# LMP88959/NTSC-CRT

Measured on AMD Instinct MI355X. Metric: frames/sec at 640x480 interlaced, bit-exact vs CPU; % HBM roofline, higher is better.
Workload: dtype int32; 1 GPU; NTSC 640x480 -> 640x480 BGRA, interlaced, full colour, noise 24, hue 0, scanlines 1 (BASELINE configs[1]); mode=independent frames (crthip_fieldpass), launch=eager, batches_in_flight=2

## Files before the change

### ntsc-crt_amd/csrc/crt_decode.hip

```cpp
#include "crt_decode_lane.h"

static int decoder_min_tier(const crthip_ctx *c, const crthip_params *p)
{
    const int b = p->bright < 0 ? -p->bright : p->bright;
    const long ct = p->contrast < 0 ? -(long) p->contrast : (long) p->contrast;
    if (c->force_exact || b > FAST_BRIGHT_MAX || ct >= (1 << 23)) return 3;
    bool coef_ok = p->eq_lf[0] >= 32768 && p->eq_lf[0] < 98304 && p->eq_hf[0] >= 32768 && p->eq_hf[0] < 98304 &&
                   p->eq_lf[1] > 0 && p->eq_lf[1] < 32768 && p->eq_hf[1] > 0 && p->eq_hf[1] < 32768 &&
                   p->eq_lf[2] > 0 && p->eq_lf[2] < 32768 && p->eq_hf[2] > 0 && p->eq_hf[2] < 32768;
    for (int cas = 0; cas < 2 && coef_ok; cas++) {
        const double cf = cas ? p->eq_hf[0] : p->eq_lf[0], al = cf / 65536.0, den = 1.0 - (al > 1.0 ? al - 1.0 : 1.0 - al);
        double prev = 127.0 + b, worst = 0.0;
        for (int k = 0; k < 4; k++) {
            const double cur = (al * prev + 1.0) / den + 1.0;
            if (prev + cur > worst) worst = prev + cur;
            prev = cur;
        }
        if (cf * worst + 32768.0 >= 2147483647.0) coef_ok = false;
    }
    if (c->no_tier0 || !coef_ok || b > T0_BRIGHT_MAX) return 2;
    const long vmax = 16380L * (10L * (127 + b) + 64) + 11551L * 3870L;
    if (((vmax >> 12) + 1) * ct >= (1L << 31)) return 2;
    return c->no_loskip ? 2 : 0;
}
// ... 34 lines not shown
                   const crthip_line *d_lines, void *d_out, size_t ostride, size_t fstride)
{
    if (!fstride) fstride = c->fstride;
    c->last_fstage = 0;
    {
        const int rc = crt_decode_check(c, p);
        if (rc) return rc;
    }
    const bool wide_px = c->px_tile ? c->px_tile >= 32 : p->outw >= 1280;
    const bool rows_shape = !p->eq_kernel && (c->shape == 2 || (c->shape == 0 && n <= ROWS_SHAPE_MAX_FIELDS &&
                            !(n >= WIDE_SHAPE_MIN_FIELDS && !p->bloom && crt_decode_wide_ok(c, p, decoder_min_tier(c, p), wide_px))));
    if (rows_shape) return crt_run_decode_rows(c, p, n, d_inp, d_lines, d_out, ostride, fstride);
    if (p->bloom) return crt_run_decode_bloom_lanes(c, p, n, d_inp, d_lines, d_out, ostride, decoder_min_tier(c, p), fstride);
    const int min_tier = p->eq_kernel ? (decoder_min_tier(c, p) == 3 ? 5 : 4) : decoder_min_tier(c, p);
    const bool wide = wide_px;
    const bool use_wide = crt_decode_wide_ok(c, p, min_tier, wide);
    FStageArgs fsa;
    const bool fstage = crt_decode_fstages(c, p, min_tier, &fsa) && !use_wide;
    c->last_fstage = fstage;
    const unsigned span = (unsigned) p->outh + p->v_fac;
    const int passes = span >= (unsigned) c->sd.lines ? 1 : (int) (((unsigned) c->sd.lines + span - 1) / (span ? span : 1));
    return dispatch_system(c->system, c->pattern, [&](auto tag) {
        using S = decltype(tag);
        {
        const int total = n * S::LINES;
        const block_order bo = make_block_order((total + 63) / 64, c->dec_order_env == -1 ? n : c->dec_order_env);
        const dim3 grid(bo.grid), block(64);
        unsigned char *o = (unsigned char *) d_out;
        ProfScope ps(c, CRTHIP_K_DECODE);
        for (int rank = 0; rank < passes; rank++) {
#define CRTHIP_LAUNCH_DECODE(TG, B3) \
    do { if constexpr (S::CCS != 4 && TG == 2) break;  \
         if constexpr (S::CCS == 4 && TG == 0) { if (fstage) {  \
             if (wide) hipLaunchKernelGGL((k_decode<S, TG, B3, 32, false, true>), grid, block, 0, c->stream, *p, n, d_inp, fstride, d_lines, o, ostride, min_tier, rank, (const int *) nullptr, bo.K, bo.per, fsa); \
             else hipLaunchKernelGGL((k_decode<S, TG, B3, 16, false, true>), grid, block, 0, c->stream, *p, n, d_inp, fstride, d_lines, o, ostride, min_tier, rank, (const int *) nullptr, bo.K, bo.per, fsa); \
             break; } } \
         if (wide) hipLaunchKernelGGL((k_decode<S, TG, B3, 32>), grid, block, 0, c->stream, *p, n, d_inp, fstride, d_lines, o, ostride, min_tier, rank, (const int *) nullptr, bo.K, bo.per, fsa); \
         else hipLaunchKernelGGL((k_decode<S, TG, B3, 16>), grid, block, 0, c->stream, *p, n, d_inp, fstride, d_lines, o, ostride, min_tier, rank, (const int *) nullptr, bo.K, bo.per, fsa); } while (0)
            if (use_wide) {
                const int rc = crt_run_decode_wide(c, p, n, d_inp, d_lines, d_out, ostride, min_tier, rank, fstride);
                if (rc) return rc;
                CRTHIP_LAUNCH_DECODE(1, false);
                continue;
            }
            if (p->out_bpp == 3) {
                if (min_tier <= 1) CRTHIP_LAUNCH_DECODE(0, true);
                if (min_tier <= 3) CRTHIP_LAUNCH_DECODE(1, true);
                if (min_tier >= 4) CRTHIP_LAUNCH_DECODE(2, true);
            } else {
                if (min_tier <= 1) CRTHIP_LAUNCH_DECODE(0, false);
                if (min_tier <= 3) CRTHIP_LAUNCH_DECODE(1, false);
                if (min_tier >= 4) CRTHIP_LAUNCH_DECODE(2, false);
            }
#undef CRTHIP_LAUNCH_DECODE
        }
        return CRTHIP_OK;
        }
    });
}
```

### ntsc-crt_amd/csrc/crt_decode3.hip

```cpp
#include "crt_decode_lane.h"

#define BLOOM_BUCKETS 256
#define BLOOM_KEY_BIAS 64

template <class S>
__device__ __forceinline__ int bloom_key(const crthip_line &lp, int outw)
{
    if ((lp.nrows & CRTHIP_LINE_NROWS_MASK) == 0) return -1;
    const int half = S::AV_LEN / 2 + 8 - (lp.scanl >> 12);
    const int line_w = 2 * half + (lp.dx != ((2 * half) << 12) / outw ? 1 : 0);
    const int key = line_w - S::AV_LEN * 112 / 128 + BLOOM_KEY_BIAS;
    return key < 0 ? 0 : key >= BLOOM_BUCKETS ? BLOOM_BUCKETS - 1 : key;
}

#define BLOOM_SORT_ROUNDS 16

template <class S>
__global__ void __launch_bounds__(256)
k_bloom_count(int total, int outw, const crthip_line *__restrict__ lines, int *__restrict__ hist)
{
    __shared__ int s_hist[BLOOM_BUCKETS];
    const int t = threadIdx.x;
    s_hist[t] = 0;
    __syncthreads();
// ... 67 lines not shown
                               const crthip_line *d_lines, void *d_out, size_t ostride, int min_tier, size_t fstride)
{
    const int total = n * c->sd.lines;
    const size_t slots = bloom_slots(c, n);
    const int rc_ = crt_reserve_bloom(c, n);
    if (rc_) return rc_;
    int *hist = c->d_bloom, *cursor = hist + BLOOM_BUCKETS, *perm = cursor + BLOOM_BUCKETS;
    const bool wide = c->px_tile ? c->px_tile >= 32 : p->outw >= 1280;
    const unsigned span = (unsigned) p->outh + p->v_fac;
    const int passes = span >= (unsigned) c->sd.lines ? 1 : (int) (((unsigned) c->sd.lines + span - 1) / (span ? span : 1));
    if (min_tier == 1 && c->sd.cc_samples != 5) min_tier = 2;
    FStageArgs fsa;
    const bool fstage = crt_decode_fstages(c, p, min_tier, &fsa);
    return dispatch_system(c->system, c->pattern, [&](auto tag) {
        using S = decltype(tag);
        if constexpr (S::NES_TIMING) {
            return set_err(c, CRTHIP_E_ARG, "no bloom build of the NES systems", hipSuccess);
        } else {
            ProfScope ps(c, CRTHIP_K_DECODE);
            {
                const size_t want = (slots + 255) / 256;
                static_assert(2 * BLOOM_BUCKETS <= 256 * 4, "the first blocks clear the histogram and the cursors");
                hipLaunchKernelGGL(k_bloom_clear, dim3((unsigned) (want < 4 ? 4 : want > 2048 ? 2048 : want)), dim3(256), 0, c->stream,
                                   hist, 2 * BLOOM_BUCKETS, perm, slots);
            }
            const dim3 sgrid((total + 256 * BLOOM_SORT_ROUNDS - 1) / (256 * BLOOM_SORT_ROUNDS)), sblock(256);
            hipLaunchKernelGGL((k_bloom_count<S>), sgrid, sblock, 0, c->stream, total, p->outw, d_lines, hist);
            hipLaunchKernelGGL((k_bloom_scatter<S>), sgrid, sblock, 0, c->stream, total, p->outw, d_lines, hist, cursor, perm);
            const dim3 grid((unsigned) (slots / 64)), block(64);
            unsigned char *o = (unsigned char *) d_out;
            for (int rank = 0; rank < passes; rank++) {
#define CRTHIP_LAUNCH_BLOOM(TG, B3) \
    do { if constexpr (S::CCS == 4 && TG == 0) { if (fstage) {  \
             if (wide) hipLaunchKernelGGL((k_decode<S, TG, B3, 32, true, true>), grid, block, 0, c->stream, *p, n, d_inp, fstride, d_lines, o, ostride, min_tier, rank, (const int *) perm, 0, 0, fsa); \
             else hipLaunchKernelGGL((k_decode<S, TG, B3, 16, true, true>), grid, block, 0, c->stream, *p, n, d_inp, fstride, d_lines, o, ostride, min_tier, rank, (const int *) perm, 0, 0, fsa); \
             break; } } \
         if (wide) hipLaunchKernelGGL((k_decode<S, TG, B3, 32, true>), grid, block, 0, c->stream, *p, n, d_inp, fstride, d_lines, o, ostride, min_tier, rank, (const int *) perm, 0, 0, fsa); \
         else hipLaunchKernelGGL((k_decode<S, TG, B3, 16, true>), grid, block, 0, c->stream, *p, n, d_inp, fstride, d_lines, o, ostride, min_tier, rank, (const int *) perm, 0, 0, fsa); } while (0)
                if (p->out_bpp == 3) {
                    if (min_tier <= 1) CRTHIP_LAUNCH_BLOOM(0, true);
                    CRTHIP_LAUNCH_BLOOM(1, true);
                } else {
                    if (min_tier <= 1) CRTHIP_LAUNCH_BLOOM(0, false);
                    CRTHIP_LAUNCH_BLOOM(1, false);
                }
#undef CRTHIP_LAUNCH_BLOOM
            }
            return CRTHIP_OK;
        }
    });
}
```

### ntsc-crt_amd/csrc/crt_decode_lane.h

```cpp
#ifndef CRT_DECODE_LANE_H
#define CRT_DECODE_LANE_H
#include "crt_dev.h"
#include <type_traits>


struct Eq3 { int lo0, lo1, lo2, lo3, hi0, hi1, hi2, hi3, h0, h1, h2; };

template <bool FAST, int G1, int G2>
__device__ __forceinline__ int eq_step(Eq3 &f, const int lf, const int hf, const int s)
{
    f.lo0 += (mulq<FAST>(lf, s - f.lo0) + 32768) >> 16;
    f.hi0 += (mulq<FAST>(hf, s - f.hi0) + 32768) >> 16;
    f.lo1 += (mulq<FAST>(lf, f.lo0 - f.lo1) + 32768) >> 16;
    f.hi1 += (mulq<FAST>(hf, f.hi0 - f.hi1) + 32768) >> 16;
    f.lo2 += (mulq<FAST>(lf, f.lo1 - f.lo2) + 32768) >> 16;
    f.hi2 += (mulq<FAST>(hf, f.hi1 - f.hi2) + 32768) >> 16;
    f.lo3 += (mulq<FAST>(lf, f.lo2 - f.lo3) + 32768) >> 16;
    f.hi3 += (mulq<FAST>(hf, f.hi2 - f.hi3) + 32768) >> 16;
    int r = (f.lo3 * 65536) >> 16;
    if (G1 == 65536 || G1 == 8192) r += ((f.hi3 - f.lo3) * G1) >> 16;
    else r += mulq<FAST>(f.hi3 - f.lo3, G1) >> 16;
    if (G2 != 0) {
        r += mulq<FAST>(f.h2 - f.hi3, G2) >> 16;
        f.h2 = f.h1; f.h1 = f.h0; f.h0 = s;
// ... 58 lines not shown
__device__ __forceinline__ void fstage_round_down(bool on)
{
    __builtin_amdgcn_sched_barrier(0);
    if (on) asm volatile("s_setreg_imm32_b32 hwreg(HW_REG_MODE, 0, 2), 2\n\ts_nop 1" ::: "memory");
    else asm volatile("s_setreg_imm32_b32 hwreg(HW_REG_MODE, 0, 2), 0\n\ts_nop 1" ::: "memory");
    __builtin_amdgcn_sched_barrier(0);
}
__device__ __forceinline__ float fbits(int b) { return __int_as_float(b); }
__device__ __forceinline__ float subf(float a, float b)
{
    float r;
    asm("v_sub_f32 %0, %1, %2" : "=v"(r) : "v"(a), "v"(b));
    return r;
}
__device__ __forceinline__ float fmaf_vs(float d, int m_uniform, float acc)
{
    float r;
    asm("v_fma_f32 %0, %1, %2, %3" : "=v"(r) : "v"(d), "s"(m_uniform), "v"(acc));
    return r;
}
__device__ __forceinline__ float addf_sv(int k_uniform, float x)
{
    float r;
    asm("v_add_f32 %0, %1, %2" : "=v"(r) : "s"(k_uniform), "v"(x));
    return r;
}
template <bool NEG> __device__ __forceinline__ float fmaf_vvs(float a, float b, int k_uniform)
{
    float r;
    if (NEG) asm("v_fma_f32 %0, %1, -%2, %3" : "=v"(r) : "v"(a), "v"(b), "s"(k_uniform));
    else asm("v_fma_f32 %0, %1, %2, %3" : "=v"(r) : "v"(a), "v"(b), "s"(k_uniform));
    return r;
}
__device__ __forceinline__ int unbias(float x, int k_uniform)
{
    int r;
    asm("v_subrev_u32 %0, %1, %2" : "=v"(r) : "s"(k_uniform), "v"(x));
    return r;
}
__device__ __forceinline__ float cvt_sbyte(int word, int k)
{
    float r;
    if (k == 0) asm("v_cvt_f32_i32_sdwa %0, sext(%1) dst_sel:DWORD dst_unused:UNUSED_PAD src0_sel:BYTE_0" : "=v"(r) : "v"(word));
    else if (k == 1) asm("v_cvt_f32_i32_sdwa %0, sext(%1) dst_sel:DWORD dst_unused:UNUSED_PAD src0_sel:BYTE_1" : "=v"(r) : "v"(word));
    else if (k == 2) asm("v_cvt_f32_i32_sdwa %0, sext(%1) dst_sel:DWORD dst_unused:UNUSED_PAD src0_sel:BYTE_2" : "=v"(r) : "v"(word));
    else asm("v_cvt_f32_i32_sdwa %0, sext(%1) dst_sel:DWORD dst_unused:UNUSED_PAD src0_sel:BYTE_3" : "=v"(r) : "v"(word));
    return r;
}
__device__ __forceinline__ void eqf_reset(EqF &f, int x0, int dstage)
{
    f.lo0 = f.hi0 = fbits(x0); f.lo1 = f.hi1 = fbits(x0 + dstage); f.lo2 = f.hi2 = fbits(x0 + 2 * dstage); f.lo3 = f.hi3 = fbits(x0 + 3 * dstage);
    f.h0 = f.h1 = f.h2 = 0;
}
template <int G1, int G2>
__device__ __forceinline__ void eq_stepf_yiq(EqF &y, EqF &ci_, EqF &cq_, const int myl, const int myh, const int mi, const int mq,
                                             const float uyl, const float uyh, const float ui, const float uq,
                                             const int kyl, const int ki, const int koyl, const int koyh, const int koi, const int koq,
                                             int &cy, int &ci, int &cq)
{
#define EQF_PIN() __builtin_amdgcn_sched_barrier(0)
    float d0 = subf(uyl, y.lo0), d1 = subf(uyh, y.hi0), d2 = subf(ui, ci_.hi0), d3 = subf(uq, cq_.hi0);
    EQF_PIN();
    y.lo0 = fmaf_vs(d0, myl, uyl); y.hi0 = fmaf_vs(d1, myh, uyh); ci_.hi0 = fmaf_vs(d2, mi, ci_.hi0); cq_.hi0 = fmaf_vs(d3, mq, cq_.hi0);
    EQF_PIN();
#define EQF_STAGES(P, N)                                                                                                         \
    d0 = subf(y.lo##P, y.lo##N); d1 = subf(y.hi##P, y.hi##N); d2 = subf(ci_.hi##P, ci_.hi##N); d3 = subf(cq_.hi##P, cq_.hi##N);   \
    EQF_PIN();                                                                                                                   \
    y.lo##N = fmaf_vs(d0, myl, y.lo##P); y.hi##N = fmaf_vs(d1, myh, y.hi##P);                                                    \
    ci_.hi##N = fmaf_vs(d2, mi, ci_.hi##N); cq_.hi##N = fmaf_vs(d3, mq, cq_.hi##N);                                              \
    EQF_PIN();
    EQF_STAGES(0, 1)
    EQF_STAGES(1, 2)
    EQF_STAGES(2, 3)
#undef EQF_STAGES
#undef EQF_PIN
    const int lo3 = unbias(y.lo3, koyl), hi3 = unbias(y.hi3, koyh);
    int r;
    if (G1 == 8192) r = lo3 + ((hi3 - lo3) >> 3);
    else r = ((lo3 * 65536) >> 16) + (__mul24(hi3 - lo3, G1) >> 16);
    r += __mul24(y.h2 - hi3, G2) >> 16;
    y.h2 = y.h1; y.h1 = y.h0; y.h0 = unbias(uyl, kyl);
    cy = r;
    const int i3 = unbias(ci_.hi3, koi);
    ci = i3 + (__mul24(ci_.h2 - i3, 1311) >> 16);
    ci_.h2 = ci_.h1; ci_.h1 = ci_.h0; ci_.h0 = unbias(ui, ki);
    cq = unbias(cq_.hi3, koq);
}

struct Fir { int p1, p2, p3, acc, r0, r1, r2, r3; };
template <int M>
__device__ __forceinline__ int fir_step(Fir &f, int x, const int K )
{
    if (M >= 1) { const int t = x + f.p1; f.p1 = x; x = t; }
    if (M >= 2) { const int t = x + f.p2; f.p2 = x; x = t; }
    if (M >= 3) { const int t = x + f.p3; f.p3 = x; x = t; }
    int &slot = K == 0 ? f.r0 : K == 1 ? f.r1 : K == 2 ? f.r2 : f.r3;
    f.acc += x - slot;
    slot = x;
    return f.acc >> (2 + M);
}

__device__ __forceinline__ unsigned pack_selector(int format)
{
    return format == CRTHIP_FMT_BGRA ? 0x03020100u : format == CRTHIP_FMT_RGBA ? 0x03000102u
         : format == CRTHIP_FMT_ARGB ? 0x00010203u : 0x02010003u ;
}
__device__ __forceinline__ unsigned unpack_selector(int format)
{
    return format == CRTHIP_FMT_BGRA ? 0x03020100u : format == CRTHIP_FMT_RGBA ? 0x03000102u
         : format == CRTHIP_FMT_ARGB ? 0x00010203u : 0x00030201u ;
}

#ifndef DEC_IN_TILE_DW
#define DEC_IN_TILE_DW 16
#endif
#ifdef DEC_WAVES_PER_EU
#define DEC_OCCUPANCY_ATTR __attribute__((amdgpu_waves_per_eu(DEC_WAVES_PER_EU, DEC_WAVES_PER_EU)))
#else
#define DEC_OCCUPANCY_ATTR
#endif
template <class S, int TG, bool BPP3, int PXT, bool BLOOM = false, bool FSTAGE = false>
__global__ void __launch_bounds__(64) DEC_OCCUPANCY_ATTR
k_decode(const crthip_params P, int n_fields, const signed char *__restrict__ inp, size_t fstride,
         const crthip_line *__restrict__ lines, unsigned char *__restrict__ outp, size_t ostride, int min_tier,
         int want_rank, const int *__restrict__ perm, int order_k, int order_per, const FStageArgs FS)
{
    static_assert(!FSTAGE || (TG == 0 && S::CCS == 4), "float stages: tiers 0 / 1 of the 4-sample systems");
    constexpr int TLO = 2 * TG;
    constexpr int IN_TILE_DW = DEC_IN_TILE_DW, IN_PIECES = IN_TILE_DW / 4;
    using TIN = TileRows<IN_TILE_DW>;
    __shared__ unsigned s_in[TIN::DWORDS];
    constexpr int PX_TILE = PXT, PX_PIECES = PXT / 4;
    using TPX = TileRows<PXT>;
    __shared__ unsigned s_px[TPX::DWORDS];
    __shared__ unsigned long long s_src[64], s_dst[64];
    __shared__ int s_nrows[64];

    const int lane = threadIdx.x;
    int gid = block_item(blockIdx.x, order_k, order_per) * 64 + lane;
    if (BLOOM) gid = perm[gid];
    const bool live = BLOOM ? gid >= 0 : gid < n_fields * S::LINES;
    crthip_line lp;
    lp.pos = 0; lp.wave0 = 0; lp.wave1 = 0; lp.beg = 0; lp.nrows = 0; lp.hsync = 0;
    const int f = live ? gid / S::LINES : 0;
    if (live) lp = lines[gid];
    int tier = __ballot(lp.nrows & CRTHIP_LINE_EXACT) ? 3 : __ballot(lp.nrows & CRTHIP_LINE_NOT64) ? 2
             : __ballot(lp.nrows & CRTHIP_LINE_WIDE) ? (BLOOM && S::CCS != 5 ? 2 : 1) : 0;
    if (tier < 2 && __ballot(lp.nrows & (int) CRTHIP_LINE_KEEPLO) != 0ull) tier = 2;
    if (min_tier >= 4) tier = (min_tier == 5 || tier == 3) ? 5 : 4;
    else if (tier < min_tier) tier = min_tier;
    if (tier != TLO && tier != TLO + 1) return;
    int nrows = lp.nrows & CRTHIP_LINE_NROWS_MASK;
    const int rank = (lp.nrows >> CRTHIP_LINE_RANK_SHIFT) & CRTHIP_LINE_RANK_MASK;
    if (!live || rank != want_rank) nrows = 0;
// ... 22 lines not shown
    s_dst[lane] = (unsigned long long) (outp + (size_t) f * ostride + (size_t) (act ? lp.beg : 0) * pitch);
    s_nrows[lane] = nrows;
    wave_lds_fence();

    constexpr int WSCALE = TIER <= 1 ? 128 : 1;
    const int w0 = lp.wave0 * WSCALE, w1 = lp.wave1 * WSCALE, nw0 = -lp.wave0 * WSCALE, nw1 = -lp.wave1 * WSCALE;
    if constexpr (S::CCS == 5) {
#pragma unroll
        for (int i = 0; i < 5; i++) {
            s_w5[lane * W5_STRIDE + 2 * i] = ((lp.wave0 * P.dem_cs[0][i] + lp.wave1 * P.dem_sn[0][i]) >> 15) * P.saturation * WSCALE;
            s_w5[lane * W5_STRIDE + 2 * i + 1] = ((lp.wave0 * P.dem_cs[1][i] + lp.wave1 * P.dem_sn[1][i]) >> 15) * P.saturation * WSCALE;
        }
    }
    const int first = scanl_u >> 12;
    const int xq0 = first >> 2;
    int ph5 = (xq0 * 4) % 5;
    constexpr int GY1 = S::CCS == 5 ? 12192 : 8192, GY2 = S::CCS == 5 ? 7775 : 9175;
    const int bright = P.bright, contrast = P.contrast;
    const int ylf = P.eq_lf[0], yhf = P.eq_hf[0], ilf = P.eq_lf[1], ihf = P.eq_hf[1], qlf = P.eq_lf[2], qhf = P.eq_hf[2];
    const unsigned psel = pack_selector(P.out_format), usel = unpack_selector(P.out_format);
    const bool rgb_order = P.out_format == CRTHIP_FMT_RGB;
    const bool blend = P.blend != 0;
    Eq3 ey = {}, ei = {}, eq = {};
    Fir fy = {}, fi = {}, fq = {};
    const int fir_m = P.eq_kernel - 4;
    Eq64 wy, wi_, wq_;
    eq64_reset(wy); eq64_reset(wi_); eq64_reset(wq_);
    const int ylfm = (ylf - 65536) << 16, yhfm = (yhf - 65536) << 16;
    const int ihfm = ihf << 16, qhfm = qhf << 16;
    EqF gy, gi, gq;
    eqf_reset(gy, FS.x0[0], FS.dstage[0]);
    gy.hi0 = fbits(FS.x0[1]); gy.hi1 = fbits(FS.x0[1] + FS.dstage[1]); gy.hi2 = fbits(FS.x0[1] + 2 * FS.dstage[1]); gy.hi3 = fbits(FS.x0[1] + 3 * FS.dstage[1]);
    eqf_reset(gi, FS.x0[2], FS.dstage[2]); eqf_reset(gq, FS.x0[3], FS.dstage[3]);
    const float wf0 = (float) lp.wave0 * (1.0f / 512.0f), wf1 = (float) lp.wave1 * (1.0f / 512.0f);
    int kin0 = FS.in0[0], kin1 = FS.in0[1], kin2 = FS.in0[2], kin3 = FS.in0[3];
    int kout0 = FS.out0[0], kout1 = FS.out0[1], kout2 = FS.out0[2], kout3 = FS.out0[3];
    int py = 0, pi = 0, pq = 0;

    const unsigned long long ppos_all = (unsigned long long) (unsigned) dx_u * (unsigned) P.outw + (unsigned) scanl_u;
    const unsigned scan_r = (unsigned) (S::AV_LEN - 1) << 12;
    const unsigned ppos_end = ppos_all < scan_r ? (unsigned) ppos_all : scan_r;
    const unsigned dx = (unsigned) dx_u;
    unsigned ppos = (unsigned) scanl_u;
    const int outw = P.outw;
    int px = 0, px0 = 0;
    int tile_end = PX_TILE < outw ? PX_TILE : outw;
    const int contrast12 = contrast * 4096;
    long alpha_pair = (long) 0xff00ul << 32;
    asm volatile("" : "+v"(alpha_pair));

    const int in_row = lane / IN_PIECES, in_piece = lane % IN_PIECES;
    constexpr int IN_ROWS = 64 / IN_PIECES;
    const int t0 = xq0 / IN_TILE_DW;
    v4i stage[IN_PIECES];
#pragma unroll
    for (int i = 0; i < IN_PIECES; i++) {
        stage[i] = gload16u(s_src[i * IN_ROWS + in_row] + t0 * (IN_TILE_DW * 4) + in_piece * 16);
    }
    constexpr int NQ = (S::AV_LEN + 3) / 4;
    constexpr int NT = (NQ + IN_TILE_DW - 1) / IN_TILE_DW;
    for (int t = t0; t < NT; t++) {
        wave_lds_fence();
#pragma unroll
        for (int i = 0; i < IN_PIECES; i++) {
            unsigned *d = s_in + TIN::row(i * IN_ROWS + in_row) + in_piece * 4;
            d[0] = (unsigned) stage[i].x; d[1] = (unsigned) stage[i].y; d[2] = (unsigned) stage[i].z; d[3] = (unsigned) stage[i].w;
        }
        wave_lds_fence();
        if (t + 1 < NT) {
#pragma unroll
            for (int i = 0; i < IN_PIECES; i++) {
                stage[i] = gload16u(s_src[i * IN_ROWS + in_row] + (t + 1) * (IN_TILE_DW * 4) + in_piece * 16);
            }
        }
        const int xq_end = (t + 1) * IN_TILE_DW < NQ ? (t + 1) * IN_TILE_DW : NQ;
        for (int xq = t == t0 ? xq0 : t * IN_TILE_DW; xq < xq_end; xq++) {
            const int word = (int) s_in[TIN::row(lane) + (xq - t * IN_TILE_DW)];
#pragma unroll
            for (int k = 0; k < 4; k++) {
                const int x = xq * 4 + k;
                const int s = (word << (24 - 8 * k)) >> 24;
                int wi = k == 0 ? w0 : k == 1 ? w1 : k == 2 ? nw0 : nw1;
                int wq = k == 0 ? nw1 : k == 1 ? w0 : k == 2 ? w1 : nw0;
                if constexpr (S::CCS == 5) {
                    wi = s_w5[lane * W5_STRIDE + 2 * ph5];
                    wq = s_w5[lane * W5_STRIDE + 2 * ph5 + 1];
                    ph5 = ph5 == 4 ? 0 : ph5 + 1;
                }
                if (BLOOM && x < first) continue;
                int cy, ci, cq;
                if (FSTAGE) {
                    const float fs = cvt_sbyte(word, k);
                    const float uyl = addf_sv(kin0 + bright, fs), uyh = addf_sv(kin1 + bright, fs);
                    const float ui = k == 0 ? fmaf_vvs<false>(fs, wf0, kin2) : k == 1 ? fmaf_vvs<false>(fs, wf1, kin2)
                                   : k == 2 ? fmaf_vvs<true>(fs, wf0, kin2) : fmaf_vvs<true>(fs, wf1, kin2);
                    const float uq = k == 0 ? fmaf_vvs<true>(fs, wf1, kin3) : k == 1 ? fmaf_vvs<false>(fs, wf0, kin3)
                                   : k == 2 ? fmaf_vvs<false>(fs, wf1, kin3) : fmaf_vvs<true>(fs, wf0, kin3);
                    eq_stepf_yiq<GY1, GY2>(gy, gi, gq, FS.mul[0], FS.mul[1], FS.mul[2], FS.mul[3], uyl, uyh, ui, uq,
                                           kin0, kin2, kout0, kout1, kout2, kout3, cy, ci, cq);
                    ci >>= 3; cq >>= 3;
                    kin0 += FS.drift[0]; kin1 += FS.drift[1]; kin2 += FS.drift[2]; kin3 += FS.drift[3];
                    kout0 += FS.drift[0]; kout1 += FS.drift[1]; kout2 += FS.drift[2]; kout3 += FS.drift[3];
                } else if (TIER == 0) {
                    eq_step64_yiq<GY1, GY2>(wy, wi_, wq_, ylfm, yhfm, ihfm, qhfm, pair_of(s + bright), __mul24(s, wi), __mul24(s, wq), cy, ci, cq);
                    ci >>= 3; cq >>= 3;
                } else if (TIER == 1) {
                    eq_step64_yiq<GY1, GY2>(wy, wi_, wq_, ylfm, yhfm, ihfm, qhfm, pair_of(s + bright), mul_lo_mad64(s, wi), mul_lo_mad64(s, wq), cy, ci, cq);
                    ci >>= 3; cq >>= 3;
                } else if (FIR) {
                    const int uy = s + bright, ui = mulq<FAST>(s, wi) >> 9, uq = mulq<FAST>(s, wq) >> 9;
#define CRT_FIR3(M) do { cy = fir_step<M>(fy, uy, k) << 4; ci = fir_step<M>(fi, ui, k) >> 3; cq = fir_step<M>(fq, uq, k) >> 3; } while (0)
                    if (fir_m == 3) CRT_FIR3(3); else if (fir_m == 2) CRT_FIR3(2); else if (fir_m == 1) CRT_FIR3(1); else CRT_FIR3(0);
#undef CRT_FIR3
                } else {
                    cy = eq_step<FAST, GY1, GY2>(ey, ylf, yhf, s + bright) << 4;
                    ci = eq_step<FAST, 65536, 1311>(ei, ilf, ihf, mulq<FAST>(s, wi) >> 9) >> 3;
                    cq = eq_step<FAST, 65536, 0>(eq, qlf, qhf, mulq<FAST>(s, wq) >> 9) >> 3;
                }
                if (BLOOM && x >= S::AV_LEN - 1) { cy = 0; ci = 0; cq = 0; }
                const unsigned lim_x = (unsigned) x << 12;
                const unsigned lim = lim_x < ppos_end ? lim_x : ppos_end;
                while (ppos < lim) {
                    const int R = (int) (ppos & 0xfffu), L = 0xfff - R;
                    int yy;
                    if (TIER <= 1) {
                        yy = mad24_vs(cy, R << 2, mulq_vs<true>(py, L << 2));
                    } else {
                        yy = (mulq_vs<FAST>(py, L) >> 2) + (mulq_vs<FAST>(cy, R) >> 2);
                    }
                    unsigned rgb;
                    if (TIER <= 1) {
                        int iq = add_hiwords(mulq_vs<true>(pq, L << 2), mulq_vs<true>(cq, R << 2));
                        iq = add_hiwords_to_hi(iq, mulq_vs<true>(pi, L << 2), mulq_vs<true>(ci, R << 2));
                        const int vr = dot2_vs(iq, (3879 << 16) | 2556, yy);
                        const int vg = dot2_vs(iq, (int) (((unsigned) -1126 << 16) | ((unsigned) -2605 & 0xffffu)), yy);
// ... 115 lines not shown
```

### ntsc-crt_amd/csrc/crt_dev.h

```cpp
#ifndef CRT_DEV_H
#define CRT_DEV_H

#include <hip/hip_runtime.h>

#include <stdint.h>
#include <stdio.h>
#include <stdlib.h>
#include <string.h>

#include <new>

#include "crt_hip.h"
#include "crt_setup.h"

struct SysCommon {
    static constexpr int VRES = 262;
    static constexpr int CCS = 4, CB_LEN = 40;
    static constexpr int VS_SEP_END = 0;
    static constexpr bool IS_NES = false;
    static constexpr bool NES_TIMING = false;
    static constexpr bool IS_VHS = false;
    static constexpr bool LINE_ROWS = false;
    static constexpr bool BANDLIMIT = true;
    static constexpr bool IIR_Y_NEAR = true;
// ... 123 lines not shown
}

#define CRTHIP_LINE_EXACT 0x40000000
#define CRTHIP_LINE_NROWS_MASK 0xffff
#define CRTHIP_LINE_RANK_SHIFT 16
#define CRTHIP_LINE_RANK_MASK  0xfff
#define CRTHIP_LINE_WIDE  0x10000000
#define CRTHIP_LINE_NOT64 0x20000000
#define CRTHIP_LINE_KEEPLO 0x80000000
#define LOSKIP_WAVE_MAX   65532
#define T0_WAVE_MAX       120000
#define T0_BRIGHT_MAX     2600
#define FAST_WAVE_MAX     524288
#define FAST_BRIGHT_MAX   130000
#define LCG_MUL 214019u
#define LCG_ADD 140327895u

template <int CCS>
__device__ __forceinline__ int line_tier_flags(int wave0, int wave1, int saturation, int loskip_wave_max, bool reads_tail)
{
    if (reads_tail && loskip_wave_max > LOSKIP_WAVE_MAX) loskip_wave_max = LOSKIP_WAVE_MAX;
    long a;
    const long a0 = wave0 < 0 ? -(long) wave0 : wave0, a1 = wave1 < 0 ? -(long) wave1 : wave1;
    if (CCS == 4) a = a0 > a1 ? a0 : a1;
    else a = (a0 + a1 + 1) * (saturation < 0 ? -(long) saturation : (long) saturation);
    if (a > FAST_WAVE_MAX) return CRTHIP_LINE_EXACT;
    if (a > T0_WAVE_MAX) return CRTHIP_LINE_NOT64;
    int f = 0;
    if (a > LOSKIP_WAVE_MAX) f |= CRTHIP_LINE_WIDE;
    if (a > loskip_wave_max) f |= (int) CRTHIP_LINE_KEEPLO;
    return f;
}

struct FStageArgs { int mul[4], x0[4], dstage[4], in0[4], out0[4], drift[4]; };

typedef int v4i __attribute__((ext_vector_type(4)));
struct __attribute__((packed)) unaligned16 { v4i v; };
struct __attribute__((packed)) unaligned4 { int v; };

typedef __attribute__((address_space(1))) unaligned16 g_unaligned16;
typedef __attribute__((address_space(1))) unsigned g_u32;
typedef __attribute__((address_space(1))) unsigned char g_u8;
__device__ __forceinline__ v4i gload16u(unsigned long long a) { return ((const g_unaligned16 *) a)->v; }
__device__ __forceinline__ void gstore16u(unsigned long long a, v4i v) { ((g_unaligned16 *) a)->v = v; }
typedef v4i v4i_a4 __attribute__((aligned(4)));
typedef __attribute__((address_space(1))) v4i_a4 g_v4i;
__device__ __forceinline__ void gstore16u_nt(unsigned long long a, v4i v) { __builtin_nontemporal_store(v, (g_v4i *) a); }
__device__ __forceinline__ v4i gload16u_nt(unsigned long long a) { return __builtin_nontemporal_load((const g_v4i *) a); }
__device__ __forceinline__ unsigned gload32(unsigned long long a) { return *(const g_u32 *) a; }
__device__ __forceinline__ void gstore32(unsigned long long a, unsigned v) { *(g_u32 *) a = v; }
__device__ __forceinline__ unsigned gload8(unsigned long long a) { return *(const g_u8 *) a; }
__device__ __forceinline__ void gstore8(unsigned long long a, unsigned v) { *(g_u8 *) a = (unsigned char) v; }

__device__ __forceinline__ v4i load16u(const void *p) { return ((const unaligned16 *) p)->v; }
__device__ __forceinline__ void store16u(void *p, v4i v) { ((unaligned16 *) p)->v = v; }
__device__ __forceinline__ int load4u(const void *p) { return ((const unaligned4 *) p)->v; }
__device__ __forceinline__ void store4u(void *p, int v) { ((unaligned4 *) p)->v = v; }

__device__ __forceinline__ void wave_lds_fence()
{
    __builtin_amdgcn_fence(__ATOMIC_RELEASE, "wavefront");
    __builtin_amdgcn_wave_barrier();
    __builtin_amdgcn_fence(__ATOMIC_ACQUIRE, "wavefront");
}

__device__ __forceinline__ int posmod(int x, int n) { return ((x % n) + n) % n; }
// ... 206 lines not shown
    int skel_yo;
    int shape;
    int row_tile;
    int sync_kernel;
    uint2 *d_jump1;
    int *d_bloom;
    size_t bloom_cap;
    unsigned char *d_seq;
    size_t seq_cap;
    int *seq_sets_host;
    size_t seq_sets_host_cap;
    bool vhs_prechained;
    int seq_guess_n;
    unsigned *d_vhs_rows;
    int vhs_chunks;
    signed char *d_vhs_dig;
    int vhs_mfma;
    int wide_decode;
    unsigned *d_vhs_hist;
    unsigned *d_vhs_next;
    int px_tile;
    int ac_tile;
    int ac_tile_env;
    int wide_lpw_env;
    int sig_pad;
    size_t fstride_pad;
    sig_layout last_lay;
    int last_n;
    signed char *d_still_sig;
    size_t still_cap;
    sig_layout still_lay;
    int wide_order_env, dec_order_env, act_order_env;
    int dec_float;
    int last_fstage;
    int sig_tile_env;
    int overlap_chunks;
    const crthip_knob_rec *knob_recs;
    int knob_loskip;
    const crthip_knob_rec *seq_knob_recs;
    crthip_knobs_env seq_knob_env;
    hipStream_t aux_stream;
    hipEvent_t ev_fork, ev_join, ev_chunk[CRTHIP_MAX_CHUNKS];
    hipEvent_t ev_mfork, ev_mjoin;
    int margin_side;
    bool prof;
    double prof_ms[CRTHIP_K_COUNT];
    int prof_n[CRTHIP_K_COUNT];
    struct Pending { int k; hipEvent_t a, b; } *pend;
    int npend, cappend;
    char err[256];
};

static inline int set_err(crthip_ctx *c, int code, const char *what, hipError_t e)
{
    if (c) snprintf(c->err, sizeof(c->err), "%s: %s", what, e == hipSuccess ? "" : hipGetErrorString(e));
    return code;
}
#define HIPCHK(ctx, call) do { hipError_t e_ = (call); if (e_ != hipSuccess) return set_err(ctx, CRTHIP_E_HIP, #call, e_); } while (0)

static inline void lcg_jump_host(unsigned k, unsigned *mul, unsigned *add)
{
    unsigned am = LCG_MUL, ac = LCG_ADD, rm = 1u, rc = 0u;
    while (k) {
        if (k & 1u) { rm = am * rm; rc = am * rc + ac; }
        ac = am * ac + ac;
        am = am * am;
// ... 108 lines not shown
```

### ntsc-crt_amd/csrc/crt_host.hip

```cpp
#include "crt_dev.h"

__global__ void k_seq_rn(int n_fields, crthip_state *state, uint2 whole_field, unsigned first_index, unsigned rn0)
{
    const int k = blockIdx.x * blockDim.x + threadIdx.x;
    if (k >= n_fields) return;
    unsigned pm = whole_field.x, pa = whole_field.y, m = 1u, a = 0u;
    for (unsigned e = first_index + (unsigned) k; e; e >>= 1) {
        if (e & 1u) { m = pm * m; a = pm * a + pa; }
        pa = pm * pa + pa;
        pm = pm * pm;
    }
    state[k].rn = (int) (m * rn0 + a);
}

__global__ void k_seq_load(int n_fields, crthip_state *state, const int2 *guess, int2 first)
{
    const int k = blockIdx.x * blockDim.x + threadIdx.x;
    if (k >= n_fields) return;
    const int2 v = k ? guess[k - 1] : first;
    state[k].hsync = v.x;
    state[k].vsync = v.y;
}

__global__ void k_seq_compare(int n_fields, const crthip_state *state, int2 *guess, int *changed)
// ... 484 lines not shown
        return CRTHIP_E_ARG;
    }
    int ndev = 0;
    if (hipGetDeviceCount(&ndev) != hipSuccess || ndev <= 0 || device < 0 || device >= ndev) return CRTHIP_E_NODEVICE;
    hipDeviceProp_t prop;
    if (hipGetDeviceProperties(&prop, device) != hipSuccess) return CRTHIP_E_NODEVICE;
    if (strncmp(prop.gcnArchName, "gfx950", 6) != 0) {
        fprintf(stderr, "crthip: device %d is %s, this library is built for gfx950 only\n", device, prop.gcnArchName);
        return CRTHIP_E_NODEVICE;
    }
    crthip_ctx *c = new (std::nothrow) crthip_ctx();
    if (!c) return CRTHIP_E_NOMEM;
    memset(c, 0, sizeof(*c));
    c->device = device; c->system = system; c->pattern = chroma_pattern; c->sd = sd;
    c->fstride = crthip_field_stride(system, chroma_pattern);
    if (hipSetDevice(device) != hipSuccess) {
        delete c;
        return CRTHIP_E_HIP;
    }
    c->stream = 0;
    c->overlap_chunks = 0;
    { const char *e = getenv("CRTHIP_SYNC_KERNEL"); c->sync_kernel = e ? atoi(e) : 0; }
    { const char *e = getenv("CRTHIP_ROW_TILE"); c->row_tile = e ? atoi(e) : 0; }
    { const char *e = getenv("CRTHIP_WIDE_DECODE"); c->wide_decode = e ? atoi(e) != 0 : 1; }
    { const char *e = getenv("CRTHIP_AC_TILE"); c->ac_tile_env = e && (atoi(e) == 16 || atoi(e) == 32) ? atoi(e) : 0; }
    { const char *e = getenv("CRTHIP_WIDE_LPW"); c->wide_lpw_env = e && (atoi(e) == 8 || atoi(e) == 16) ? atoi(e) : 0; }
    { const char *e = getenv("CRTHIP_MARGIN_SIDE"); c->margin_side = e ? atoi(e) != 0 : 1; }
    { const char *e = getenv("CRTHIP_SIG_PAD"); c->sig_pad = e ? atoi(e) != 0 : 1; }
    c->fstride_pad = 0;
    dispatch_system(system, chroma_pattern, [&](auto tag) { c->fstride_pad = PadGeom<decltype(tag)>::FSTRIDE; return CRTHIP_OK; });
    { const char *e = getenv("CRTHIP_WIDE_ORDER"); c->wide_order_env = e ? atoi(e) : 0; }
    { const char *e = getenv("CRTHIP_DEC_ORDER"); c->dec_order_env = e ? atoi(e) : 0; }
    { const char *e = getenv("CRTHIP_ACT_ORDER"); c->act_order_env = e ? atoi(e) : 0; }
    { const char *e = getenv("CRTHIP_DEC_FLOAT"); c->dec_float = e ? atoi(e) != 0 : 1; c->last_fstage = 0; }
    { const char *e = getenv("CRTHIP_SIG_TILE"); c->sig_tile_env = e && (atoi(e) == 16 || atoi(e) == 32 || atoi(e) == 64) ? atoi(e) : 0; }
    c->own_stream = false;
    const int nq = sd.input_size / 16 + 2;
    uint2 *h = (uint2 *) malloc(sizeof(uint2) * (size_t) nq);
    if (!h) { crthip_destroy(c); return CRTHIP_E_NOMEM; }
    unsigned m16, a16;
    lcg_jump_host(16, &m16, &a16);
    h[0].x = 1u; h[0].y = 0u;
    for (int q = 1; q < nq; q++) { h[q].x = m16 * h[q - 1].x; h[q].y = m16 * h[q - 1].y + a16; }
    lcg_jump_host((unsigned) sd.input_size, &c->whole_field.x, &c->whole_field.y);
    if (hipMalloc((void **) &c->d_jump16, sizeof(uint2) * (size_t) nq) != hipSuccess ||
        hipMemcpy(c->d_jump16, h, sizeof(uint2) * (size_t) nq, hipMemcpyHostToDevice) != hipSuccess) {
        free(h);
        crthip_destroy(c);
        return CRTHIP_E_HIP;
    }
    free(h);
    if (system == CRTHIP_SYSTEM_NES && (hipMalloc((void **) &c->d_nes_tab, NES_TAB_SIZE) != hipSuccess ||
                                        hipMalloc((void **) &c->d_nes_tab_alt, NES_TAB_SIZE) != hipSuccess)) {
        crthip_destroy(c);
        return CRTHIP_E_NOMEM;
    }
    {
        uint2 j1[16];
        j1[0] = make_uint2(1u, 0u);
        for (int k = 1; k < 16; k++) j1[k] = make_uint2(LCG_MUL * j1[k - 1].x, LCG_MUL * j1[k - 1].y + LCG_ADD);
        if (hipMalloc((void **) &c->d_skel, (size_t) SKEL_VARIANTS * c->fstride) != hipSuccess ||
            hipMalloc((void **) &c->d_skel_alt, (size_t) SKEL_VARIANTS * c->fstride) != hipSuccess ||
            hipMalloc((void **) &c->d_jump1, sizeof(j1)) != hipSuccess ||
            hipMemcpy(c->d_jump1, j1, sizeof(j1), hipMemcpyHostToDevice) != hipSuccess) {
            crthip_destroy(c);
            return CRTHIP_E_NOMEM;
// ... 1171 lines not shown
```

Measured before the change: 1.721 million frames/sec.

## Add packed-f32 equaliser path and integer history for float-stage decode

Adds a packed two-lane float variant of the decoder's four-stage equaliser using v_pk_fma_f32/v_pk_add_f32, selectable via CRTHIP_DEC_PACKED (default off). It also moves the per-band history into integer registers (FHist), folding the unbias subtractions and the I-band rounding constant into precomputed terms, so the default scalar float path changes too. The aim is fewer VALU instructions per sample in the decode inner loop. The packed path needs exact bit-compatibility and may raise register pressure.

Result: no change. 1.710 million frames/sec (-0.6%).

```diff
diff --git a/ntsc-crt_amd/csrc/crt_decode.hip b/ntsc-crt_amd/csrc/crt_decode.hip
--- a/ntsc-crt_amd/csrc/crt_decode.hip
+++ b/ntsc-crt_amd/csrc/crt_decode.hip
@@ -90,8 +90,10 @@
 #define CRTHIP_LAUNCH_DECODE(TG, B3) \
     do { if constexpr (S::CCS != 4 && TG == 2) break;  \
          if constexpr (S::CCS == 4 && TG == 0) { if (fstage) {  \
-             if (wide) hipLaunchKernelGGL((k_decode<S, TG, B3, 32, false, true>), grid, block, 0, c->stream, *p, n, d_inp, fstride, d_lines, o, ostride, min_tier, rank, (const int *) nullptr, bo.K, bo.per, fsa); \
-             else hipLaunchKernelGGL((k_decode<S, TG, B3, 16, false, true>), grid, block, 0, c->stream, *p, n, d_inp, fstride, d_lines, o, ostride, min_tier, rank, (const int *) nullptr, bo.K, bo.per, fsa); \
+             if (wide && c->dec_packed) hipLaunchKernelGGL((k_decode<S, TG, B3, 32, false, 2>), grid, block, 0, c->stream, *p, n, d_inp, fstride, d_lines, o, ostride, min_tier, rank, (const int *) nullptr, bo.K, bo.per, fsa); \
+             else if (wide) hipLaunchKernelGGL((k_decode<S, TG, B3, 32, false, 1>), grid, block, 0, c->stream, *p, n, d_inp, fstride, d_lines, o, ostride, min_tier, rank, (const int *) nullptr, bo.K, bo.per, fsa); \
+             else if (c->dec_packed) hipLaunchKernelGGL((k_decode<S, TG, B3, 16, false, 2>), grid, block, 0, c->stream, *p, n, d_inp, fstride, d_lines, o, ostride, min_tier, rank, (const int *) nullptr, bo.K, bo.per, fsa); \
+             else hipLaunchKernelGGL((k_decode<S, TG, B3, 16, false, 1>), grid, block, 0, c->stream, *p, n, d_inp, fstride, d_lines, o, ostride, min_tier, rank, (const int *) nullptr, bo.K, bo.per, fsa); \
              break; } } \
          if (wide) hipLaunchKernelGGL((k_decode<S, TG, B3, 32>), grid, block, 0, c->stream, *p, n, d_inp, fstride, d_lines, o, ostride, min_tier, rank, (const int *) nullptr, bo.K, bo.per, fsa); \
          else hipLaunchKernelGGL((k_decode<S, TG, B3, 16>), grid, block, 0, c->stream, *p, n, d_inp, fstride, d_lines, o, ostride, min_tier, rank, (const int *) nullptr, bo.K, bo.per, fsa); } while (0)
diff --git a/ntsc-crt_amd/csrc/crt_decode3.hip b/ntsc-crt_amd/csrc/crt_decode3.hip
--- a/ntsc-crt_amd/csrc/crt_decode3.hip
+++ b/ntsc-crt_amd/csrc/crt_decode3.hip
@@ -123,8 +123,8 @@
             for (int rank = 0; rank < passes; rank++) {
 #define CRTHIP_LAUNCH_BLOOM(TG, B3) \
     do { if constexpr (S::CCS == 4 && TG == 0) { if (fstage) {  \
-             if (wide) hipLaunchKernelGGL((k_decode<S, TG, B3, 32, true, true>), grid, block, 0, c->stream, *p, n, d_inp, fstride, d_lines, o, ostride, min_tier, rank, (const int *) perm, 0, 0, fsa); \
-             else hipLaunchKernelGGL((k_decode<S, TG, B3, 16, true, true>), grid, block, 0, c->stream, *p, n, d_inp, fstride, d_lines, o, ostride, min_tier, rank, (const int *) perm, 0, 0, fsa); \
+             if (wide) hipLaunchKernelGGL((k_decode<S, TG, B3, 32, true, 1>), grid, block, 0, c->stream, *p, n, d_inp, fstride, d_lines, o, ostride, min_tier, rank, (const int *) perm, 0, 0, fsa); \
+             else hipLaunchKernelGGL((k_decode<S, TG, B3, 16, true, 1>), grid, block, 0, c->stream, *p, n, d_inp, fstride, d_lines, o, ostride, min_tier, rank, (const int *) perm, 0, 0, fsa); \
              break; } } \
          if (wide) hipLaunchKernelGGL((k_decode<S, TG, B3, 32, true>), grid, block, 0, c->stream, *p, n, d_inp, fstride, d_lines, o, ostride, min_tier, rank, (const int *) perm, 0, 0, fsa); \
          else hipLaunchKernelGGL((k_decode<S, TG, B3, 16, true>), grid, block, 0, c->stream, *p, n, d_inp, fstride, d_lines, o, ostride, min_tier, rank, (const int *) perm, 0, 0, fsa); } while (0)
diff --git a/ntsc-crt_amd/csrc/crt_decode_lane.h b/ntsc-crt_amd/csrc/crt_decode_lane.h
--- a/ntsc-crt_amd/csrc/crt_decode_lane.h
+++ b/ntsc-crt_amd/csrc/crt_decode_lane.h
@@ -114,12 +114,7 @@
     else asm("v_fma_f32 %0, %1, %2, %3" : "=v"(r) : "v"(a), "v"(b), "s"(k_uniform));
     return r;
 }
-__device__ __forceinline__ int unbias(float x, int k_uniform)
-{
-    int r;
-    asm("v_subrev_u32 %0, %1, %2" : "=v"(r) : "s"(k_uniform), "v"(x));
-    return r;
-}
+__device__ __forceinline__ int fint(float x) { return __float_as_int(x); }
 __device__ __forceinline__ float cvt_sbyte(int word, int k)
 {
     float r;
@@ -134,10 +129,33 @@
     f.lo0 = f.hi0 = fbits(x0); f.lo1 = f.hi1 = fbits(x0 + dstage); f.lo2 = f.hi2 = fbits(x0 + 2 * dstage); f.lo3 = f.hi3 = fbits(x0 + 3 * dstage);
     f.h0 = f.h1 = f.h2 = 0;
 }
+struct FHist { int y0, y1, y2, i0, i1, i2; };
+__device__ __forceinline__ void eqf_hist_reset(FHist &h, int kin_i, int drift_i)
+{
+    h.y0 = h.y1 = h.y2 = 0;
+    h.i0 = kin_i - drift_i; h.i1 = kin_i - 2 * drift_i; h.i2 = kin_i - 3 * drift_i;
+}
 template <int G1, int G2>
-__device__ __forceinline__ void eq_stepf_yiq(EqF &y, EqF &ci_, EqF &cq_, const int myl, const int myh, const int mi, const int mq,
-                                             const float uyl, const float uyh, const float ui, const float uq,
-                                             const int kyl, const int ki, const int koyl, const int koyh, const int koi, const int koq,
+__device__ __forceinline__ void eqf_bands(FHist &h, const float flo3, const float fhi3, const float fi3, const float fq3, const float ui,
+                                          const int sb, const int koyl, const int koyh, const int nkoi, const int koq, const int topk,
+                                          int &cy, int &ci, int &cq)
+{
+    const int lo3 = fint(flo3) - koyl, hi3 = fint(fhi3) - koyh;
+    int r;
+    if (G1 == 8192) r = lo3 + ((hi3 - lo3) >> 3);
+    else r = ((lo3 * 65536) >> 16) + (__mul24(hi3 - lo3, G1) >> 16);
+    r += __mul24(h.y2 - hi3, G2) >> 16;
+    h.y2 = h.y1; h.y1 = h.y0; h.y0 = sb;
+    cy = r;
+    const int ib = fint(fi3);
+    ci = ib + ((__mul24(h.i2 - ib, 1311) + topk) >> 16) + nkoi;
+    h.i2 = h.i1; h.i1 = h.i0; h.i0 = fint(ui);
+    cq = fint(fq3) - koq;
+}
+template <int G1, int G2>
+__device__ __forceinline__ void eq_stepf_yiq(EqF &y, EqF &ci_, EqF &cq_, FHist &h, const int myl, const int myh, const int mi, const int mq,
+                                             const float uyl, const float uyh, const float ui, const float uq, const int sb,
+                                             const int koyl, const int koyh, const int nkoi, const int koq, const int topk,
                                              int &cy, int &ci, int &cq)
 {
 #define EQF_PIN() __builtin_amdgcn_sched_barrier(0)
@@ -156,17 +174,58 @@
     EQF_STAGES(2, 3)
 #undef EQF_STAGES
 #undef EQF_PIN
-    const int lo3 = unbias(y.lo3, koyl), hi3 = unbias(y.hi3, koyh);
-    int r;
-    if (G1 == 8192) r = lo3 + ((hi3 - lo3) >> 3);
-    else r = ((lo3 * 65536) >> 16) + (__mul24(hi3 - lo3, G1) >> 16);
-    r += __mul24(y.h2 - hi3, G2) >> 16;
-    y.h2 = y.h1; y.h1 = y.h0; y.h0 = unbias(uyl, kyl);
-    cy = r;
-    const int i3 = unbias(ci_.hi3, koi);
-    ci = i3 + (__mul24(ci_.h2 - i3, 1311) >> 16);
-    ci_.h2 = ci_.h1; ci_.h1 = ci_.h0; ci_.h0 = unbias(ui, ki);
-    cq = unbias(cq_.hi3, koq);
+    eqf_bands<G1, G2>(h, y.lo3, y.hi3, ci_.hi3, cq_.hi3, ui, sb, koyl, koyh, nkoi, koq, topk, cy, ci, cq);
+}
+
+typedef float v2f __attribute__((ext_vector_type(2)));
+struct EqP { v2f a0, a1, a2, a3, b0, b1, b2, b3; };
+__device__ __forceinline__ long spair(int lo, int hi) { return (long) (((unsigned long) (unsigned) hi << 32) | (unsigned) lo); }
+__device__ __forceinline__ v2f pk_subf(v2f a, v2f b)
+{
+    v2f r;
+    asm("v_pk_add_f32 %0, %1, %2 neg_lo:[0,1] neg_hi:[0,1]" : "=v"(r) : "v"(a), "v"(b));
+    return r;
+}
+__device__ __forceinline__ v2f pk_fmaf_vs(v2f d, long m_uniform, v2f acc)
+{
+    v2f r;
+    asm("v_pk_fma_f32 %0, %1, %2, %3" : "=v"(r) : "v"(d), "s"(m_uniform), "v"(acc));
+    return r;
+}
+__device__ __forceinline__ v2f pk_addf_sv_lo(long k_uniform, v2f x)
+{
+    v2f r;
+    asm("v_pk_add_f32 %0, %1, %2 op_sel_hi:[1,0]" : "=v"(r) : "s"(k_uniform), "v"(x));
+    return r;
+}
+__device__ __forceinline__ void eqp_reset(EqP &f, const FStageArgs &FS)
+{
+#define EQP_INIT(J) f.a##J = (v2f) { fbits(FS.x0[0] + J * FS.dstage[0]), fbits(FS.x0[1] + J * FS.dstage[1]) }; \
+                    f.b##J = (v2f) { fbits(FS.x0[2] + J * FS.dstage[2]), fbits(FS.x0[3] + J * FS.dstage[3]) };
+    EQP_INIT(0) EQP_INIT(1) EQP_INIT(2) EQP_INIT(3)
+#undef EQP_INIT
+}
+template <int G1, int G2>
+__device__ __forceinline__ void eq_steppk_yiq(EqP &f, FHist &h, const long ma, const long mb, const v2f ua, const v2f ub, const int sb,
+                                              const int koyl, const int koyh, const int nkoi, const int koq, const int topk,
+                                              int &cy, int &ci, int &cq)
+{
+#define EQP_PIN() __builtin_amdgcn_sched_barrier(0)
+    v2f da = pk_subf(ua, f.a0), db = pk_subf(ub, f.b0);
+    EQP_PIN();
+    f.a0 = pk_fmaf_vs(da, ma, ua); f.b0 = pk_fmaf_vs(db, mb, f.b0);
+    EQP_PIN();
+#define EQP_STAGES(P, N)                                                                                                         \
+    da = pk_subf(f.a##P, f.a##N); db = pk_subf(f.b##P, f.b##N);                                                                  \
+    EQP_PIN();                                                                                                                   \
+    f.a##N = pk_fmaf_vs(da, ma, f.a##P); f.b##N = pk_fmaf_vs(db, mb, f.b##N);                                                    \
+    EQP_PIN();
+    EQP_STAGES(0, 1)
+    EQP_STAGES(1, 2)
+    EQP_STAGES(2, 3)
+#undef EQP_STAGES
+#undef EQP_PIN
+    eqf_bands<G1, G2>(h, f.a3.x, f.a3.y, f.b3.x, f.b3.y, ub.x, sb, koyl, koyh, nkoi, koq, topk, cy, ci, cq);
 }
 
 struct Fir { int p1, p2, p3, acc, r0, r1, r2, r3; };
@@ -201,7 +260,7 @@
 #else
 #define DEC_OCCUPANCY_ATTR
 #endif
-template <class S, int TG, bool BPP3, int PXT, bool BLOOM = false, bool FSTAGE = false>
+template <class S, int TG, bool BPP3, int PXT, bool BLOOM = false, int FSTAGE = 0>
 __global__ void __launch_bounds__(64) DEC_OCCUPANCY_ATTR
 k_decode(const crthip_params P, int n_fields, const signed char *__restrict__ inp, size_t fstride,
          const crthip_line *__restrict__ lines, unsigned char *__restrict__ outp, size_t ostride, int min_tier,
@@ -290,9 +349,16 @@
     eqf_reset(gy, FS.x0[0], FS.dstage[0]);
     gy.hi0 = fbits(FS.x0[1]); gy.hi1 = fbits(FS.x0[1] + FS.dstage[1]); gy.hi2 = fbits(FS.x0[1] + 2 * FS.dstage[1]); gy.hi3 = fbits(FS.x0[1] + 3 * FS.dstage[1]);
     eqf_reset(gi, FS.x0[2], FS.dstage[2]); eqf_reset(gq, FS.x0[3], FS.dstage[3]);
+    EqP gp;
+    eqp_reset(gp, FS);
+    FHist gh;
+    eqf_hist_reset(gh, FS.in0[2], FS.drift[2]);
+    const long mul_a = spair(FS.mul[0], FS.mul[1]), mul_b = spair(FS.mul[2], FS.mul[3]);
     const float wf0 = (float) lp.wave0 * (1.0f / 512.0f), wf1 = (float) lp.wave1 * (1.0f / 512.0f);
-    int kin0 = FS.in0[0], kin1 = FS.in0[1], kin2 = FS.in0[2], kin3 = FS.in0[3];
-    int kout0 = FS.out0[0], kout1 = FS.out0[1], kout2 = FS.out0[2], kout3 = FS.out0[3];
+    int kinb0 = FS.in0[0] + bright, kinb1 = FS.in0[1] + bright, kin2 = FS.in0[2], kin3 = FS.in0[3];
+    int kout0 = FS.out0[0], kout1 = FS.out0[1], nkout2 = -FS.out0[2], kout3 = FS.out0[3];
+    int topk = (3 * FS.drift[2] + FS.out0[2] - FS.in0[2]) * 1311;
+    asm volatile("" : "+v"(topk));
     int py = 0, pi = 0, pq = 0;
 
     const unsigned long long ppos_all = (unsigned long long) (unsigned) dx_u * (unsigned) P.outw + (unsigned) scanl_u;
@@ -349,16 +415,23 @@
                 int cy, ci, cq;
                 if (FSTAGE) {
                     const float fs = cvt_sbyte(word, k);
-                    const float uyl = addf_sv(kin0 + bright, fs), uyh = addf_sv(kin1 + bright, fs);
                     const float ui = k == 0 ? fmaf_vvs<false>(fs, wf0, kin2) : k == 1 ? fmaf_vvs<false>(fs, wf1, kin2)
                                    : k == 2 ? fmaf_vvs<true>(fs, wf0, kin2) : fmaf_vvs<true>(fs, wf1, kin2);
                     const float uq = k == 0 ? fmaf_vvs<true>(fs, wf1, kin3) : k == 1 ? fmaf_vvs<false>(fs, wf0, kin3)
                                    : k == 2 ? fmaf_vvs<false>(fs, wf1, kin3) : fmaf_vvs<true>(fs, wf0, kin3);
-                    eq_stepf_yiq<GY1, GY2>(gy, gi, gq, FS.mul[0], FS.mul[1], FS.mul[2], FS.mul[3], uyl, uyh, ui, uq,
-                                           kin0, kin2, kout0, kout1, kout2, kout3, cy, ci, cq);
+                    if constexpr (FSTAGE == 2) {
+                        const v2f fs1 = { fs, __builtin_nondeterministic_value(fs) };
+                        const v2f ua = pk_addf_sv_lo(spair(kinb0, kinb1), fs1);
+                        const v2f ub = { ui, uq };
+                        eq_steppk_yiq<GY1, GY2>(gp, gh, mul_a, mul_b, ua, ub, s + bright, kout0, kout1, nkout2, kout3, topk, cy, ci, cq);
+                    } else {
+                        const float uyl = addf_sv(kinb0, fs), uyh = addf_sv(kinb1, fs);
+                        eq_stepf_yiq<GY1, GY2>(gy, gi, gq, gh, FS.mul[0], FS.mul[1], FS.mul[2], FS.mul[3], uyl, uyh, ui, uq, s + bright,
+                                               kout0, kout1, nkout2, kout3, topk, cy, ci, cq);
+                    }
                     ci >>= 3; cq >>= 3;
-                    kin0 += FS.drift[0]; kin1 += FS.drift[1]; kin2 += FS.drift[2]; kin3 += FS.drift[3];
-                    kout0 += FS.drift[0]; kout1 += FS.drift[1]; kout2 += FS.drift[2]; kout3 += FS.drift[3];
+                    kinb0 += FS.drift[0]; kinb1 += FS.drift[1]; kin2 += FS.drift[2]; kin3 += FS.drift[3];
+                    kout0 += FS.drift[0]; kout1 += FS.drift[1]; nkout2 -= FS.drift[2]; kout3 += FS.drift[3];
                 } else if (TIER == 0) {
                     eq_step64_yiq<GY1, GY2>(wy, wi_, wq_, ylfm, yhfm, ihfm, qhfm, pair_of(s + bright), __mul24(s, wi), __mul24(s, wq), cy, ci, cq);
                     ci >>= 3; cq >>= 3;
diff --git a/ntsc-crt_amd/csrc/crt_dev.h b/ntsc-crt_amd/csrc/crt_dev.h
--- a/ntsc-crt_amd/csrc/crt_dev.h
+++ b/ntsc-crt_amd/csrc/crt_dev.h
@@ -179,6 +179,9 @@
     return f;
 }
 
+#ifndef CRTHIP_DEC_PACKED_DEFAULT
+#define CRTHIP_DEC_PACKED_DEFAULT 0
+#endif
 struct FStageArgs { int mul[4], x0[4], dstage[4], in0[4], out0[4], drift[4]; };
 
 typedef int v4i __attribute__((ext_vector_type(4)));
@@ -451,6 +454,7 @@
     sig_layout still_lay;
     int wide_order_env, dec_order_env, act_order_env;
     int dec_float;
+    int dec_packed;
     int last_fstage;
     int sig_tile_env;
     int overlap_chunks;
diff --git a/ntsc-crt_amd/csrc/crt_host.hip b/ntsc-crt_amd/csrc/crt_host.hip
--- a/ntsc-crt_amd/csrc/crt_host.hip
+++ b/ntsc-crt_amd/csrc/crt_host.hip
@@ -540,6 +540,7 @@
     { const char *e = getenv("CRTHIP_WIDE_ORDER"); c->wide_order_env = e ? atoi(e) : 0; }
     { const char *e = getenv("CRTHIP_DEC_ORDER"); c->dec_order_env = e ? atoi(e) : 0; }
     { const char *e = getenv("CRTHIP_ACT_ORDER"); c->act_order_env = e ? atoi(e) : 0; }
+    { const char *e = getenv("CRTHIP_DEC_PACKED"); c->dec_packed = e ? atoi(e) != 0 : CRTHIP_DEC_PACKED_DEFAULT; }
     { const char *e = getenv("CRTHIP_DEC_FLOAT"); c->dec_float = e ? atoi(e) != 0 : 1; c->last_fstage = 0; }
     { const char *e = getenv("CRTHIP_SIG_TILE"); c->sig_tile_env = e && (atoi(e) == 16 || atoi(e) == 32 || atoi(e) == 64) ? atoi(e) : 0; }
     c->own_stream = false;
```
